# Francis-Rings/MotionEditor

Measured on AMD Instinct MI355X. Metric: denoise-steps/sec, 24f x 512^2 two-branch UNet3D+ControlNet(+adapter+K/V injection), higher is better.
Workload: dtype f16

## Files before the change

motioneditor_amd/csrc/gemm.hip:

```cpp
#include "me_common.h"
#include "../../include/motioned.h"
#include <stdio.h>
#include <stdlib.h>

namespace {

constexpr int BK = 64;
#ifndef WIDE_TERMS
#define WIDE_TERMS 0
#endif
constexpr int STAGE_REG = 0, STAGE_GLDS = 1, STAGE_BUF = 2;
constexpr int ROWEPI_FLAG = 1 << 30, TILEORDER_FLAG = 1 << 29;

template <bool NT = false>
__device__ __forceinline__ void st16(f16* p, uint4 v) {
  if constexpr (NT) {
    typedef unsigned u32x4 __attribute__((ext_vector_type(4)));
    __builtin_nontemporal_store((u32x4){v.x, v.y, v.z, v.w}, reinterpret_cast<u32x4*>(p));
  } else {
    *reinterpret_cast<uint4*>(p) = v;
  }
}
template <bool NT = false>
__device__ __forceinline__ void st8(f16* p, uint2 v) {
// ... 770 lines not shown
    const int wrows = min(a.N - n0, BN);
    const auto wsrd = __builtin_amdgcn_make_buffer_rsrc(const_cast<f16*>(W + (long)n0 * wtaps * a.K), 0, (unsigned)(((long)(wrows - 1) * wtaps + taps) * a.K * 2), 0x00020000);
    unsigned xo[XROWS], wo[WROWS];
#pragma unroll
    for (int i = 0; i < WROWS; ++i) wo[i] = (unsigned)(((long)(srow + RSTR * i) * wtaps * a.K + scol) * 2);
    auto set_tap_off = [&](int tap) {
#pragma unroll
      for (int i = 0; i < XROWS; ++i) {
        const int sr = src_row(a, rinfo[i], tap, ups3);
        xo[i] = sr < 0 ? OOB : (unsigned)(((long)(sr - brow) * a.ldx + scol) * 2);
      }
    };
    int tap_l = it0 / nkc, kc_l = it0 - (it0 / nkc) * nkc;
    set_tap_off(tap_l);
    auto gload = [&](int buf) {
      char* dx = reinterpret_cast<char*>(sX + buf * BM * LD) + wave * 1024;
      char* dw = reinterpret_cast<char*>(sW + buf * BN * LD) + wave * 1024;
      const int sx = kc_l * (BK * 2), sw = (tap_l * a.K + kc_l * BK) * 2;
#pragma unroll
      for (int i = 0; i < XROWS; ++i) __builtin_amdgcn_raw_ptr_buffer_load_lds(xsrd, (lptr_t)(dx + i * (RSTR * 128)), 16, (int)xo[i], sx, 0, 0);
#pragma unroll
      for (int i = 0; i < WROWS; ++i) __builtin_amdgcn_raw_ptr_buffer_load_lds(wsrd, (lptr_t)(dw + i * (RSTR * 128)), 16, (int)wo[i], sw, 0, 0);
      if (++kc_l == nkc) {
        kc_l = 0;
        if (++tap_l < taps) set_tap_off(tap_l);
      }
    };
    gload(0);
    __syncthreads();
    for (int it = it0; it < it1; ++it) {
      const int buf = (it - it0) & 1;
      if (it + 1 < it1) gload(buf ^ 1);
      compute(buf);
      __syncthreads();
    }
    if (S > 1) {
      float* wk = reinterpret_cast<float*>(a.work) + (long)blockIdx.y * a.M * a.N;
#pragma unroll
      for (int i = 0; i < MT; ++i) {
        const int m = m0 + wm * WM + i * 16 + (lane & 15);
        if (m >= a.M) continue;
#pragma unroll
        for (int j = 0; j < NT; ++j) {
          const int n = n0 + wn * WN + j * 16 + (lane >> 4) * 4;
          if (n < a.N) *reinterpret_cast<f32x4*>(wk + (long)m * a.N + n) = acc[j][i];
        }
      }
      return;
    }
  } else if constexpr (STAGE == STAGE_GLDS) {
    typedef const __attribute__((address_space(1))) void* gptr_t;
    typedef __attribute__((address_space(3))) void* lptr_t;
    const f16* zsrc = reinterpret_cast<const f16*>(&g_zero16);
    auto gload = [&](int it, int buf) {
      int tap = it / nkc;
      int c = (it - tap * nkc) * BK + scol;
      bool kok = c < a.K;
      long wk = (long)tap * a.K + c;
      if (packk) {
        wk = it * BK + scol;
        tap = (int)wk / a.K;
        c = (int)wk - tap * a.K;
        kok = tap < 9;
        if (!kok) tap = 8;
      }
      set_tap(tap);
      char* dx = reinterpret_cast<char*>(sX + buf * BM * LD) + wave * 1024;
      char* dw = reinterpret_cast<char*>(sW + buf * BN * LD) + wave * 1024;
#pragma unroll
      for (int i = 0; i < XROWS; ++i) {
        const f16* src = (kok && xoff[i] >= 0) ? X + xoff[i] + c : zsrc;
        __builtin_amdgcn_global_load_lds((gptr_t)src, (lptr_t)(dx + i * (RSTR * 128)), 16, 0, 0);
      }
#pragma unroll
      for (int i = 0; i < WROWS; ++i) {
        const int n = n0 + srow + RSTR * i;
        const f16* src = (kok && n < a.N) ? W + (long)n * wtaps * a.K + wk : zsrc;
        __builtin_amdgcn_global_load_lds((gptr_t)src, (lptr_t)(dw + i * (RSTR * 128)), 16, 0, 0);
      }
    };
    gload(0, 0);
    __syncthreads();
    for (int it = 0; it < nit; ++it) {
      const int buf = it & 1;
      if (it + 1 < nit) gload(it + 1, buf ^ 1);
      compute(buf);
      __syncthreads();
    }
  } else {
    uint4 rx[XROWS], rw[WROWS];
    auto gload = [&](int it) {
      const int tap = it / nkc;
      const int c = (it - tap * nkc) * BK + scol;
      set_tap(tap);
      const bool kok = c < a.K;
#pragma unroll
      for (int i = 0; i < XROWS; ++i) rx[i] = (kok && xoff[i] >= 0) ? ldg128(X + xoff[i] + c) : zero128();
#pragma unroll
      for (int i = 0; i < WROWS; ++i) {
        const int n = n0 + srow + RSTR * i;
        rw[i] = (kok && n < a.N) ? ldg128(W + ((long)n * wtaps + tap) * a.K + c) : zero128();
      }
    };
    auto sstore = [&](int buf) {
      f16* dx = sX + buf * BM * LD;
      f16* dw = sW + buf * BN * LD;
#pragma unroll
      for (int i = 0; i < XROWS; ++i) *reinterpret_cast<uint4*>(dx + (srow + RSTR * i) * LD + scol) = rx[i];
#pragma unroll
      for (int i = 0; i < WROWS; ++i) *reinterpret_cast<uint4*>(dw + (srow + RSTR * i) * LD + scol) = rw[i];
    };
    gload(0);
    sstore(0);
    __syncthreads();
    for (int it = 0; it < nit; ++it) {
      const int buf = it & 1;
      if (it + 1 < nit) gload(it + 1);
      compute(buf);
      if (it + 1 < nit) sstore(buf ^ 1);
      __syncthreads();
    }
  }

  if (a.ln_stats) ln_fold_acc<NT, MT>(a, acc, m0 + wm * WM, n0 + wn * WN, lane);
  const int ncols = a.geglu ? BN / 2 : BN;
  const int Nout = a.geglu ? a.N / 2 : a.N;
  constexpr bool CFITS = (size_t)BM * (BN + 8) <= (size_t)2 * (BM + BN) * LD;
  const bool wide_store = CFITS && (Nout % 8 == 0) && (a.ldc % 8 == 0) && ((reinterpret_cast<uintptr_t>(a.C) & 15) == 0) && !a.C2 && !ups3;
  auto rowfn = [&](int i) {
    const int m = m0 + wm * WM + i * 16 + (lane & 15);
    if (m >= a.M) return -1;
    return ups3 ? out_row(a, make_row(a, m, par, true), par) : m;
  };
  if (!wide_store) {
    epilogue<NT, MT, WN>(a, acc, rowfn, m0, n0, wn, lane, nullptr, 0);
    return;
  }
  constexpr int CLD = BN + 8;
  f16* sC = reinterpret_cast<f16*>(smem);
  epilogue<NT, MT, WN>(a, acc, rowfn, m0, n0, wn, lane, sC, CLD);
  __syncthreads();
  f16* C = reinterpret_cast<f16*>(a.C);
  const int vpr = ncols / 8;
  const int nb0 = a.geglu ? n0 / 2 : n0;
  for (int idx = tid; idx < BM * vpr; idx += NTHR) {
    const int row = idx / vpr, c8 = (idx - row * vpr) * 8;
    const int m = m0 + row, n = nb0 + c8;
    if (m < a.M && n < Nout) *reinterpret_cast<uint4*>(C + (long)m * a.ldc + n) = *reinterpret_cast<const uint4*>(sC + row * CLD + c8);
  }
}

constexpr int HALO_W = 18, HALO_ROWS = HALO_W * HALO_W, HALO_INSTR = (HALO_ROWS + 7) / 8;
constexpr int HALO_BYTES = HALO_INSTR * 1024, CONVW_BYTES = 320 * 128;

__global__ __launch_bounds__(512, 2) void conv3_halo_kernel(const me_gemm_args a) {
  constexpr int BN = 320, WN = 160, NT = 10, MT = 4;
  extern __shared__ __attribute__((aligned(16))) char smem[];
  char* sH = smem;
  char* sWt = smem + HALO_BYTES;

  const int tid = threadIdx.x;
  const int lane = tid & 63;
  const int wave = __builtin_amdgcn_readfirstlane(tid >> 6);
  const int wm = wave >> 1, wn = wave & 1;

  const int nbn = a.N / BN;
  const int tx_n = a.Win >> 4, ppi = tx_n * (a.Hin >> 4);
  const int hw = a.Hin * a.Win;
  const int w = xcd_remap(blockIdx.x, (a.M / hw) * ppi * nbn);
  const int tile_n = w % nbn, patch = w / nbn;
  const int img = patch / ppi, pr = patch - img * ppi;
  const int ty = pr / tx_n, tx = pr - ty * tx_n;
  const int y0 = ty * 16, x0 = tx * 16, n0 = tile_n * BN;

  const f16* __restrict__ X = reinterpret_cast<const f16*>(a.X);
  const f16* __restrict__ W = reinterpret_cast<const f16*>(a.W);

  const int srow = wave * 8 + (lane >> 3);
  const int scol = ((lane & 7) ^ ((4 * (wave & 1) + (lane >> 4)) & 7)) * 8;
  typedef __attribute__((address_space(3))) void* lptr_t;
  constexpr unsigned OOB = 0x80000000u;
  const auto xsrd = __builtin_amdgcn_make_buffer_rsrc(const_cast<f16*>(X + (long)img * hw * a.ldx), 0, OOB, 0x00020000);
  const auto wsrd = __builtin_amdgcn_make_buffer_rsrc(const_cast<f16*>(W + (long)n0 * 9 * a.K), 0, (unsigned)((long)BN * 9 * a.K * 2), 0x00020000);
  unsigned hoff[6];
#pragma unroll
  for (int i = 0; i < 6; ++i) {
    const int hr = srow + 64 * i;
    unsigned o = OOB;
    if (hr < HALO_ROWS) {
      const int hy = hr / HALO_W, hx = hr - hy * HALO_W;
      const int iy = y0 - 1 + hy, ix = x0 - 1 + hx;
      if (iy >= 0 && iy < a.Hin && ix >= 0 && ix < a.Win) o = (unsigned)(((long)(iy * a.Win + ix) * a.ldx + scol) * 2);
    }
    hoff[i] = o;
  }
  auto load_halo = [&](int kc) {
#pragma unroll
    for (int i = 0; i < 6; ++i) {
      if (wave + 8 * i < HALO_INSTR)
        __builtin_amdgcn_raw_ptr_buffer_load_lds(xsrd, (lptr_t)(sH + (wave + 8 * i) * 1024), 16, (int)hoff[i], kc * (BK * 2), 0, 0);
    }
  };
  unsigned woff[5];
#pragma unroll
  for (int i = 0; i < 5; ++i) woff[i] = (unsigned)(((long)(srow + 64 * i) * 9 * a.K + scol) * 2);
  auto load_w = [&](int tap, int kc, int buf) {
    char* dw = sWt + buf * CONVW_BYTES + wave * 1024;
    const int so = (tap * a.K + kc * BK) * 2;
#pragma unroll
    for (int i = 0; i < 5; ++i) __builtin_amdgcn_raw_ptr_buffer_load_lds(wsrd, (lptr_t)(dw + i * 8192), 16, (int)woff[i], so, 0, 0);
  };

  f32x4 acc[NT][MT];
  init_acc<NT, MT, WN>(a, acc, n0, wn, lane);

  const int frow = lane & 15, fg = lane >> 4;
  auto compute = [&](int tap, int buf) {
    const int ky = tap / 3, kx = tap - ky * 3;
    const char* bw = sWt + buf * CONVW_BYTES;
    const int hbase = (wm * 4 + ky) * HALO_W + kx + frow;
#pragma unroll
    for (int ks = 0; ks < BK / 32; ++ks) {
      f16x8 fx[MT], fw[NT];
#pragma unroll
      for (int i = 0; i < MT; ++i) {
        const int row = hbase + i * HALO_W;
        fx[i] = *reinterpret_cast<const f16x8*>(sH + row * 128 + (((ks * 4 + fg) ^ ((row >> 1) & 7)) << 4));
      }
#pragma unroll
      for (int j = 0; j < NT; ++j) {
        const int row = wn * WN + j * 16 + frow;
        fw[j] = *reinterpret_cast<const f16x8*>(bw + row * 128 + (((ks * 4 + fg) ^ ((row >> 1) & 7)) << 4));
      }
#pragma unroll
      for (int j = 0; j < NT; ++j)
#pragma unroll
        for (int i = 0; i < MT; ++i) acc[j][i] = mfma16(fw[j], fx[i], acc[j][i]);
    }
  };

  const int nkc = a.K / BK;
  load_halo(0);
  load_w(0, 0, 0);
  __syncthreads();
  int it = 0;
  for (int kc = 0; kc < nkc; ++kc) {
    for (int tap = 0; tap < 9; ++tap, ++it) {
      const int buf = it & 1;
      const bool last_tap = tap == 8;
      if (!last_tap) load_w(tap + 1, kc, buf ^ 1);
      else if (kc + 1 < nkc) load_w(0, kc + 1, buf ^ 1);
      compute(tap, buf);
      if (last_tap && kc + 1 < nkc) {
        __syncthreads();
        load_halo(kc + 1);
      }
      __syncthreads();
    }
  }

  auto rowfn = [&](int i) { return img * hw + (y0 + wm * 4 + i) * a.Win + x0 + (lane & 15); };
  epilogue<NT, MT, WN>(a, acc, rowfn, 0, n0, wn, lane, nullptr, 0);
}

template <int BM, int BN, bool GATHER, int EPI, bool UPS3 = false>
__global__ __launch_bounds__(512, 2) void gemm8p_kernel(const me_gemm_args a) {
  static_assert(!UPS3 || (GATHER && BN == 320 && EPI <= 0), "ups 3: gather kernels, term-free row pass or direct epilogues");
  constexpr int WN = BN / 4, NT = WN / 16, NT0 = (NT + 1) / 2, NT1 = NT / 2;
  constexpr int GR = BM / 2, HALF = GR / 2, MH = HALF / 16, MT = 2 * MH;
  constexpr int NPA = 2 * HALF / 8;
  constexpr int ABYTES = BM * 128, BUFBYTES = (BM + BN) * 128;
  static_assert(BN % 64 == 0 && NT1 >= 1 && HALF % 16 == 0 && NPA >= 8 && NPA <= 16, "wave tile");
  extern __shared__ __attribute__((aligned(16))) char smem[];

  const int tid = threadIdx.x;
  const int lane = tid & 63;
  const int wave = __builtin_amdgcn_readfirstlane(tid >> 6);
  const int wr = wave >> 2, wc = wave & 3;

  const int nbn = (a.N + BN - 1) / BN;
  const int nbm = (a.M - a.m_off + BM - 1) / BM;
  constexpr bool ups3 = UPS3;
  const int nbmp = ups3 ? 4 * nbm : nbm;
  const int w = xcd_remap(blockIdx.x, nbmp * nbn);
  int tile_n, tile_m;
  if (a.splits_ & TILEORDER_FLAG) { tile_m = w % nbmp; tile_n = w / nbmp; }
  else { tile_n = w % nbn; tile_m = w / nbn; }
  const int par = ups3 ? tile_m / nbm : 0;
  tile_m -= par * nbm;
  const int m0 = a.m_off + tile_m * BM, n0 = tile_n * BN;

  const f16* __restrict__ X = reinterpret_cast<const f16*>(a.X);
  const int taps = !GATHER ? 1 : (a.gather == ME_GATHER_CONV3 ? (ups3 ? 4 : 9) : (a.gather == ME_GATHER_TCONV ? 3 : 1));
  const int wtaps = ups3 ? 16 : taps;
  const f16* __restrict__ W = reinterpret_cast<const f16*>(a.W) + (long)(4 * par) * a.K;
  const int nkc = a.K / BK;
  const int nit = taps * nkc;

  typedef __attribute__((address_space(3))) void* lptr_t;
  constexpr unsigned OOB = 0x80000000u;
  long brow = m0;
  if (GATHER) {
    if (a.gather == ME_GATHER_CONV3) brow = (long)(m0 / (ups3 ? a.Hin * a.Win : a.Hout * a.Wout)) * a.Hin * a.Win;
    else if (a.gather == ME_GATHER_TCONV) brow = m0 > a.npix ? m0 - a.npix : 0;
  }
  const auto xsrd = __builtin_amdgcn_make_buffer_rsrc(const_cast<f16*>(X + brow * a.ldx), 0, OOB, 0x00020000);
  const int wrows = min(a.N - n0, BN);
  const auto wsrd = __builtin_amdgcn_make_buffer_rsrc(const_cast<f16*>(W + (long)n0 * wtaps * a.K), 0, (unsigned)(((long)(wrows - 1) * wtaps + taps) * a.K * 2), 0x00020000);

  const int prow = lane >> 3;
  const int scol = ((lane & 7) ^ ((4 * (wave & 1) + (lane >> 4)) & 7)) * 8;
  int rA[2][2], rB0[NT0], rB1[NT1];
#pragma unroll
  for (int i = 0; i < 2; ++i) {
    const int p = wave + 8 * i;
    rA[0][i] = __builtin_amdgcn_readfirstlane((p / (HALF / 8)) * GR + 8 * (p % (HALF / 8)));
    rA[1][i] = __builtin_amdgcn_readfirstlane((p / (HALF / 8)) * GR + HALF + 8 * (p % (HALF / 8)));
  }
  const bool two_a = __builtin_amdgcn_readfirstlane(wave + 8 < NPA ? 1 : 0) != 0;
#pragma unroll
  for (int i = 0; i < NT0; ++i) {
    const int p = wave + 8 * i;
    rB0[i] = __builtin_amdgcn_readfirstlane((p / (2 * NT0)) * WN + 8 * (p % (2 * NT0)));
  }
#pragma unroll
  for (int i = 0; i < NT1; ++i) {
    const int p = wave + 8 * i;
    rB1[i] = __builtin_amdgcn_readfirstlane((p / (2 * NT1)) * WN + 16 * NT0 + 8 * (p % (2 * NT1)));
  }

  unsigned* tab = reinterpret_cast<unsigned*>(smem + 2 * BUFBYTES);
  unsigned xo[2][2];
  if constexpr (GATHER) {
    const int r = tid & 255;
    const RowInfo ri = make_row(a, r < BM ? m0 + r : a.M, par, ups3);
    for (int tap = tid >> 8; tap < taps; tap += 2) {
      const int sr = src_row(a, ri, tap, ups3);
      tab[tap * 256 + r] = sr < 0 ? OOB : (unsigned)((long)(sr - brow) * a.ldx * 2);
    }
    if (ups3 && tid < 256) tab[4 * 256 + r] = ri.valid ? (unsigned)out_row(a, ri, par) : ~0u;
    __syncthreads();
  } else {
#pragma unroll
    for (int h = 0; h < 2; ++h)
#pragma unroll
      for (int i = 0; i < 2; ++i) {
        const int m = m0 + rA[h][i] + prow;
        xo[h][i] = (m < a.M && (i == 0 || two_a)) ? (unsigned)(((long)(m - brow) * a.ldx + scol) * 2) : OOB;
      }
  }
  unsigned wo0[NT0], wo1[NT1];
#pragma unroll
  for (int i = 0; i < NT0; ++i) wo0[i] = (unsigned)(((long)(rB0[i] + prow) * wtaps * a.K + scol) * 2);
#pragma unroll
  for (int i = 0; i < NT1; ++i) wo1[i] = (unsigned)(((long)(rB1[i] + prow) * wtaps * a.K + scol) * 2);

  struct Cur { int tap, kc, tl; };
  Cur cA0 = {0, 0, 0}, cA1 = {0, 0, 0};
  int tB0 = 0, tB1 = 0;
  auto issueA = [&](Cur& c, int half) {
    char* base = smem + (c.tl & 1) * BUFBYTES;
    const int sx = __builtin_amdgcn_readfirstlane((GATHER ? c.kc : c.tl) * (BK * 2));
    const bool live = c.tl < nit;
    unsigned v[2];
#pragma unroll
    for (int i = 0; i < 2; ++i) {
      if constexpr (GATHER) v[i] = tab[__builtin_amdgcn_readfirstlane(min(c.tap, taps - 1)) * 256 + min(rA[half][i] + prow, 255)] + (unsigned)(scol * 2);
      else v[i] = xo[half][i];
    }
    __builtin_amdgcn_raw_ptr_buffer_load_lds(xsrd, (lptr_t)(base + rA[half][0] * 128), 16, (int)(live ? v[0] : OOB), sx, 0, 0);
    if (BM == 256 || two_a) __builtin_amdgcn_raw_ptr_buffer_load_lds(xsrd, (lptr_t)(base + rA[half][1] * 128), 16, (int)(live ? v[1] : OOB), sx, 0, 0);
    ++c.tl;
    if constexpr (GATHER) {
      if (++c.kc == nkc) { c.kc = 0; ++c.tap; }
    }
  };
  auto issueB0 = [&]() {
    char* base = smem + (tB0 & 1) * BUFBYTES + ABYTES;
    const int sw = __builtin_amdgcn_readfirstlane(tB0 * (BK * 2));
    const bool live = tB0 < nit;
#pragma unroll
    for (int i = 0; i < NT0; ++i)
      __builtin_amdgcn_raw_ptr_buffer_load_lds(wsrd, (lptr_t)(base + rB0[i] * 128), 16, (int)(live ? wo0[i] : OOB), sw, 0, 0);
    ++tB0;
  };
  auto issueB1 = [&]() {
    char* base = smem + (tB1 & 1) * BUFBYTES + ABYTES;
    const int sw = __builtin_amdgcn_readfirstlane(tB1 * (BK * 2));
    const bool live = tB1 < nit;
#pragma unroll
    for (int i = 0; i < NT1; ++i)
      __builtin_amdgcn_raw_ptr_buffer_load_lds(wsrd, (lptr_t)(base + rB1[i] * 128), 16, (int)(live ? wo1[i] : OOB), sw, 0, 0);
    ++tB1;
  };

  f32x4 acc[NT][MT];
  init_acc<NT, MT, WN>(a, acc, n0, wc, lane);

  const int frow = lane & 15, fg = lane >> 4;
  const int c0 = (fg ^ ((frow >> 1) & 7)) << 4;
  const int la0 = (wr * GR + frow) * 128 + c0, la1 = la0 ^ 64;
  const int lb0 = ABYTES + (wc * WN + frow) * 128 + c0, lb1 = lb0 ^ 64;
  f16x8 fa[2][MH], fb[2][NT0];
  auto readA = [&](int buf, int half) {
#pragma unroll
    for (int i = 0; i < MH; ++i) {
      fa[0][i] = *reinterpret_cast<const f16x8*>(smem + buf * BUFBYTES + la0 + (half * MH + i) * 2048);
      fa[1][i] = *reinterpret_cast<const f16x8*>(smem + buf * BUFBYTES + la1 + (half * MH + i) * 2048);
    }
  };
  auto readB = [&](int buf, int j0, int nj) {
#pragma unroll
    for (int j = 0; j < NT0; ++j) {
      if (j < nj) {
        fb[0][j] = *reinterpret_cast<const f16x8*>(smem + buf * BUFBYTES + lb0 + (j0 + j) * 2048);
// ... 258 lines not shown
  const char* e = getenv("ME_GEMM_8P_128");
  const long v = e ? atol(e) : 192;
  return v > 0 ? v : (1L << 60);
}

long geglu_min_tiles() {
  const char* e = getenv("ME_GEMM_GEGLU_MIN");
  return e ? atol(e) : 240;
}

int min_ktiles_192() {
  const char* e = getenv("ME_GEMM_192_MINK");
  return e ? atoi(e) : 4;
}

long n64_below() {
  const char* e = getenv("ME_GEMM_N64_BELOW");
  return e ? atol(e) : 200;
}

bool tile160() {
  static int on = -1;
  if (on < 0) {
    const char* e = getenv("ME_GEMM_TILE160");
    on = (e && e[0] == '0') ? 0 : 1;
  }
  return on == 1;
}

}

extern "C" void me_set_error(const char* msg);
extern "C" void me_set_kernel(const char* name);
extern "C" const char* me_last_kernel(void);

static thread_local bool g_ln_fused = false;

template <int BM, int BN, int STAGE, int WM = 64, bool UPS3 = false>
static int launch_gemm(const me_gemm_args* a, hipStream_t st) {
  const size_t lds = (size_t)2 * (BM + BN) * (STAGE != STAGE_REG ? BK : BK + 8) * sizeof(f16);
  static bool attr_set_dev[64] = {};
  int dev_id = 0;
  (void)hipGetDevice(&dev_id);
  bool& attr_set = attr_set_dev[dev_id & 63];
  if (!attr_set) {
    if (hipFuncSetAttribute(reinterpret_cast<const void*>(&gemm_kernel<BM, BN, STAGE, WM, UPS3>), hipFuncAttributeMaxDynamicSharedMemorySize, (int)lds) != hipSuccess) {
      me_set_error("me_gemm: hipFuncSetAttribute(MaxDynamicSharedMemorySize) failed");
      return ME_EHIP;
    }
    attr_set = true;
  }
  constexpr int pm = UPS3 ? 4 : 1;
  if (UPS3 != (a->gather == ME_GATHER_CONV3 && a->ups == 3)) { me_set_error("me_gemm: internal: ups = 3 launch on the wrong instantiation"); return ME_EINVAL; }
  const int nbm = (a->M - a->m_off + BM - 1) / BM * pm, nbn = (a->N + BN - 1) / BN;
  (void)hipGetLastError();
  me_gemm_args b = *a;
  b.splits_ = 0;
  int S = 1;
  if (STAGE == STAGE_BUF && a->work) {
    const int nit = (a->K / 64) * (a->gather == ME_GATHER_CONV3 ? 9 : (a->gather == ME_GATHER_TCONV ? 3 : 1));
    const int Msel = a->sel_rows > a->M ? a->sel_rows : a->M;
    S = choose_split(a, (long)((Msel + BM - 1) / BM) * nbn, nit);
    if ((int64_t)S * a->M * a->N * 4 > a->work_bytes || a->N % 4 || ((uintptr_t)a->work & 15)) S = 1;
  }
  if (S > 1) {
    b.splits_ = S;
    hipLaunchKernelGGL((gemm_kernel<BM, BN, STAGE, WM, UPS3>), dim3(nbm * nbn, S), dim3(BM / WM * 128), lds, st, b);
    const long vec = (long)a->M * (a->N / 4);
    hipLaunchKernelGGL(gemm_splitk_reduce_kernel, dim3((unsigned)((vec + 255) / 256 < 4096 ? (vec + 255) / 256 : 4096)), dim3(256), 0, st, b);
  } else {
    hipLaunchKernelGGL((gemm_kernel<BM, BN, STAGE, WM, UPS3>), dim3(nbm * nbn), dim3(BM / WM * 128), lds, st, b);
  }
  {
    char nm[64];
    snprintf(nm, sizeof(nm), "gemm_kernel<%d,%d%s>%s", BM, BN, STAGE == STAGE_REG ? ",reg" : "", S > 1 ? "+splitk" : "");
    me_set_kernel(nm);
  }
  if (hipGetLastError() != hipSuccess) {
    me_set_error("me_gemm: kernel launch failed");
    return ME_EHIP;
  }
  return ME_OK;
}

template <int BM, int BN, bool GATHER, int EPI, bool UPS3 = false>
static int launch_gemm8p_epi(const me_gemm_args& b, hipStream_t st) {
  const int lds = 2 * (BM + BN) * 128 + (GATHER ? 9 * 256 * 4 : (EPI == 0 ? LN_LDS_BYTES : 0));
  static bool attr_set_dev[64] = {};
  int dev_id = 0;
  (void)hipGetDevice(&dev_id);
  bool& attr_set = attr_set_dev[dev_id & 63];
  if (!attr_set) {
    if (hipFuncSetAttribute(reinterpret_cast<const void*>(&gemm8p_kernel<BM, BN, GATHER, EPI, UPS3>), hipFuncAttributeMaxDynamicSharedMemorySize, lds) != hipSuccess) {
      me_set_error("me_gemm: hipFuncSetAttribute(MaxDynamicSharedMemorySize) failed");
      return ME_EHIP;
    }
    attr_set = true;
  }
  constexpr int pm = UPS3 ? 4 : 1;
  const int nbm = (b.M - b.m_off + BM - 1) / BM * pm, nbn = (b.N + BN - 1) / BN;
  hipLaunchKernelGGL((gemm8p_kernel<BM, BN, GATHER, EPI, UPS3>), dim3(nbm * nbn), dim3(512), lds, st, b);
  return ME_OK;
}

template <int BM, int BN, bool GATHER>
static int launch_gemm8p(const me_gemm_args* a, hipStream_t st) {
  (void)hipGetLastError();
  me_gemm_args b = *a;
  b.splits_ = 0;
  int epi = -1;
  {
    auto al = [](const void* p, int ld) { return p == nullptr || (ld % 8 == 0 && (reinterpret_cast<uintptr_t>(p) & 15) == 0); };
    const int f = (a->rowvec ? 2 : 0) | (a->res ? 4 : 0) | (a->res2 ? 8 : 0);
    const bool ups3 = a->gather == ME_GATHER_CONV3 && a->ups == 3;
    if (BN == 320 && !(ups3 && f != 0) && row_epilogue() && !a->geglu && a->act == 0 && a->N % 320 == 0 && (f == 0 || f == 2 || f == 4 || f == 6 || f == 12) && al(a->C, a->ldc) &&
        al(a->rowvec, a->ldrv) && al(a->res, a->ldr) && al(a->res2, a->ldr2) && (!a->C2 || f == 0))
      epi = f;
    if (tile_order_exp()) b.splits_ |= TILEORDER_FLAG;
    if (BN == 256 && BM == 256 && row_epilogue() && a->geglu && a->N % 256 == 0 && al(a->C, a->ldc) && !a->C2) epi = 0;
    if (epi >= 0) b.splits_ |= ROWEPI_FLAG;
    g_ln_fused = BN == 320 && epi >= 0 && a->ln_out != nullptr;
    if (!g_ln_fused) b.ln_out = nullptr;
  }
  int rc;
  const bool ups3_launch = a->gather == ME_GATHER_CONV3 && a->ups == 3;
  if (ups3_launch) {
    if constexpr (GATHER && BN == 320) rc = epi == 0 ? launch_gemm8p_epi<BM, BN, true, 0, true>(b, st) : launch_gemm8p_epi<BM, BN, true, -1, true>(b, st);
    else { me_set_error("me_gemm: internal: ups = 3 launch on a kernel without the mode"); return ME_EINVAL; }
  } else if constexpr (BN == 256) {
    rc = epi == 0 ? launch_gemm8p_epi<BM, BN, GATHER, 0>(b, st) : launch_gemm8p_epi<BM, BN, GATHER, -1>(b, st);
  } else {
    switch (epi) {
      case 0: rc = launch_gemm8p_epi<BM, BN, GATHER, 0>(b, st); break;
      case 2: rc = launch_gemm8p_epi<BM, BN, GATHER, 2>(b, st); break;
      case 4: rc = launch_gemm8p_epi<BM, BN, GATHER, 4>(b, st); break;
      case 6: rc = launch_gemm8p_epi<BM, BN, GATHER, 6>(b, st); break;
      case 12: rc = launch_gemm8p_epi<BM, BN, GATHER, 12>(b, st); break;
      default: rc = launch_gemm8p_epi<BM, BN, GATHER, -1>(b, st); break;
    }
  }
  if (rc != ME_OK) return rc;
  {
    char nm[64];
    snprintf(nm, sizeof(nm), "gemm8p_kernel<%d,%d,%s>", BM, BN, GATHER ? "true" : "false");
    me_set_kernel(nm);
  }
  if (hipGetLastError() != hipSuccess) {
    me_set_error("me_gemm: kernel launch failed");
    return ME_EHIP;
  }
  return ME_OK;
}

static int launch_conv_halo(const me_gemm_args* a, hipStream_t st) {
  const int lds = HALO_BYTES + 2 * CONVW_BYTES;
  static bool attr_set_dev[64] = {};
  int dev_id = 0;
  (void)hipGetDevice(&dev_id);
  bool& attr_set = attr_set_dev[dev_id & 63];
  if (!attr_set) {
    if (hipFuncSetAttribute(reinterpret_cast<const void*>(&conv3_halo_kernel), hipFuncAttributeMaxDynamicSharedMemorySize, lds) != hipSuccess) {
      me_set_error("me_gemm: hipFuncSetAttribute(MaxDynamicSharedMemorySize) failed");
      return ME_EHIP;
    }
    attr_set = true;
  }
  const long blocks = (long)(a->M / 256) * (a->N / 320);
  (void)hipGetLastError();
  hipLaunchKernelGGL(conv3_halo_kernel, dim3((unsigned)blocks), dim3(512), lds, st, *a);
  me_set_kernel("conv3_halo_kernel");
  if (hipGetLastError() != hipSuccess) {
    me_set_error("me_gemm: kernel launch failed");
    return ME_EHIP;
  }
  return ME_OK;
}

extern "C" int64_t me_gemm_work_bytes(const me_gemm_args* a) {
  if (!a || a->M <= 0 || a->N <= 0 || a->K <= 0 || a->geglu || a->K % 64 || a->N % 4) return 0;
  const int nit = (a->K / 64) * (a->gather == ME_GATHER_CONV3 ? 9 : (a->gather == ME_GATHER_TCONV ? 3 : 1));
  const long blocks = (long)((a->M + 127) / 128) * ((a->N + 159) / 160);
  const int S = choose_split(a, blocks, nit);
  return S > 1 ? (int64_t)4 * a->M * a->N * 4 : 0;
}

static int gemm_dispatch(const me_gemm_args* a, void* stream);

extern "C" int me_gemm(const me_gemm_args* a, void* stream) {
  if (!a || !a->X || !a->W || !a->C) { me_set_error("me_gemm: null pointer"); return ME_EINVAL; }
  if (a->ln_stats) {
    if (a->gather != ME_GATHER_DENSE || a->bias || a->alpha != 1.0f || a->rowvec || a->res || a->res2 || a->act || !a->ln_colsum || !a->ln_cvec || a->ln_parts < 1 || a->ln_parts > 4 || a->ln_stride < 2 * (int64_t)a->M ||
        (a->ln_stride & 1) || ((uintptr_t)a->ln_stats & 7) || (((uintptr_t)a->ln_colsum | (uintptr_t)a->ln_cvec) & 15) || !(a->ln_eps > 0.f)) {
      me_set_error("me_gemm: a LayerNorm-folded launch is dense, has no bias (it is inside ln_cvec), no rowvec / residual / activation and alpha == 1; ln_colsum / ln_cvec fp32 [N] 16-byte aligned, "
                   "ln_stats 8-byte aligned with 1 <= ln_parts <= 4 parts ln_stride >= 2 M floats apart, ln_eps > 0");
      return ME_EINVAL;
    }
  }
  if (a->ln_out && (a->geglu || a->C2 || a->N % 8 || a->N > 1536 || a->ldc % 8 || ((uintptr_t)a->C & 15) || ((uintptr_t)a->ln_out & 7) || a->ln_out_stride < 2 * (int64_t)a->M || (a->ln_out_stride & 1))) {
    me_set_error("me_gemm: ln_out needs a plain fp16 output of N % 8 == 0, N <= 1536 columns (no GEGLU, no head-major panels), ldc % 8 == 0, and parts >= 2 M floats apart");
    return ME_EINVAL;
  }
  g_ln_fused = false;
  const int rc = gemm_dispatch(a, stream);
  if (rc != ME_OK || !a->ln_out || g_ln_fused) return rc;
  char nm[96];
  snprintf(nm, sizeof(nm), "%s", me_last_kernel());
  const int rc2 = me_ln_stats(reinterpret_cast<const f16*>(a->C) + (long)a->m_off * a->ldc, a->ldc, (int64_t)a->M - a->m_off, a->N,
                              reinterpret_cast<float*>(a->ln_out) + 2 * (long)a->m_off, a->ln_out_stride, stream);
  me_set_kernel(nm);
  return rc2;
}

static int gemm_dispatch(const me_gemm_args* a, void* stream) {
  if (a->M <= 0 || a->N <= 0 || a->K <= 0) { me_set_error("me_gemm: non-positive dimension"); return ME_EINVAL; }
  if (a->K % 8 || a->ldx % 8 || a->ldc % 4 || a->N % 4) { me_set_error("me_gemm: K, ldx must be multiples of 8 and N, ldc of 4"); return ME_EINVAL; }
  if (((uintptr_t)a->X | (uintptr_t)a->W) & 15 || ((uintptr_t)a->C & 7)) { me_set_error("me_gemm: misaligned pointer"); return ME_EINVAL; }
  if (a->gather < 0 || a->gather > 2) { me_set_error("me_gemm: bad gather mode"); return ME_EINVAL; }
  if (a->gather == ME_GATHER_CONV3) {
    if (a->Hin <= 0 || a->Win <= 0 || a->Hout <= 0 || a->Wout <= 0 || (a->stride != 1 && a->stride != 2) || a->ups < 0 || a->ups > 3 ||
        (a->pad0 != 0 && a->pad0 != 1) || a->M % (a->Hout * a->Wout)) { me_set_error("me_gemm: bad conv geometry"); return ME_EINVAL; }
    if (a->ups == 3 && (a->stride != 1 || a->pad0 || a->Hout != 2 * a->Hin || a->Wout != 2 * a->Win || a->geglu)) {
      me_set_error("me_gemm: ups = 3 (folded nearest 2x) needs stride 1, pad0 = 0, Hout = 2 Hin, Wout = 2 Win and weights [N, 16, K]");
      return ME_EINVAL;
    }
  }
  if (a->gather == ME_GATHER_TCONV) {
    const int ftot = a->frames_total > 0 ? a->frames_total : a->frames;
    if (a->frames <= 0 || a->npix <= 0 || a->chunk <= 0 || ftot % a->chunk || (a->m_off == 0 && a->sel_rows <= a->M && a->M % (a->frames * a->npix)) || a->frame0 < 0 ||
        a->frame0 + a->frames > ftot) { me_set_error("me_gemm: bad tconv geometry"); return ME_EINVAL; }
  }
  if (a->rowvec && (a->rows_per_vec <= 0 || a->ldrv % 4 || ((uintptr_t)a->rowvec & 7))) { me_set_error("me_gemm: bad rowvec"); return ME_EINVAL; }
  if (a->res && (a->ldr % 4 || ((uintptr_t)a->res & 7))) { me_set_error("me_gemm: bad residual"); return ME_EINVAL; }
  if (a->res2 && (a->ldr2 % 4 || ((uintptr_t)a->res2 & 7))) { me_set_error("me_gemm: bad second residual"); return ME_EINVAL; }
  if (a->res_rows < 0 || a->res2_rows < 0) { me_set_error("me_gemm: negative res_rows"); return ME_EINVAL; }
  if (a->act < 0 || a->act > 2) { me_set_error("me_gemm: bad activation"); return ME_EINVAL; }
  if (a->bias && ((uintptr_t)a->bias & 7)) { me_set_error("me_gemm: misaligned bias"); return ME_EINVAL; }
  if (a->geglu && (a->N % 32 || a->rowvec || a->res || a->res2 || a->act || a->alpha != 1.0f)) { me_set_error("me_gemm: geglu needs N % 32 == 0, alpha == 1 and no rowvec/res/act"); return ME_EINVAL; }
  if (a->m_off < 0 || a->m_off >= a->M || (a->m_off > 0 && a->gather == ME_GATHER_CONV3)) { me_set_error("me_gemm: m_off must lie in [0, M) and is for dense / TemporalConv launches"); return ME_EINVAL; }
  if (a->C2 && (a->geglu || a->act || a->rowvec || a->res || a->res2 || a->c2_dh <= 0 || a->c2_dh % 8 || a->c2_col0 < 0 || a->c2_col0 % 16 || a->c2_col0 >= a->N ||
                (a->N - a->c2_col0) % a->c2_dh || a->c2_hs % 8 || a->c2_hs < (int64_t)a->M * a->c2_dh || ((uintptr_t)a->C2 & 15) || a->gather == ME_GATHER_CONV3)) {
    me_set_error("me_gemm: head-major output (C2) needs a term-free epilogue, c2_dh % 8 == 0, c2_col0 % 16 == 0, whole heads, c2_hs % 8 == 0 and >= M * c2_dh, 16-byte alignment");
    return ME_EINVAL;
  }
  hipStream_t st = reinterpret_cast<hipStream_t>(stream);
  me_gemm_args par_args;
  const int pm = a->gather == ME_GATHER_CONV3 && a->ups == 3 ? 4 : 1;
  if (pm == 4) {
    par_args = *a;
    par_args.M = a->M / 4;
    par_args.sel_rows = a->sel_rows / 4;
    par_args.ln_out = nullptr;
    a = &par_args;
  }
#define ME_LAUNCH_GEMM(BM_, BN_, STAGE_) (pm == 4 ? launch_gemm<BM_, BN_, STAGE_, 64, true>(a, st) : launch_gemm<BM_, BN_, STAGE_>(a, st))
  const bool wide = a->N % 128 == 0 || a->N % 64 != 0;
  if (stage_impl() == STAGE_GLDS || pm == 4) {
    const int Msel = a->sel_rows > a->M ? a->sel_rows : a->M;
    const long big_blocks = (long)((Msel + 255) / 256) * pm * (a->N / 320);
    if (a->gather == ME_GATHER_CONV3 && a->stride == 1 && a->ups == 0 && !a->pad0 && a->N % 320 == 0 && a->K % 64 == 0 && a->Hin % 16 == 0 &&
        a->Win % 16 == 0 && !a->geglu && big_blocks >= halo_min_blocks() && conv_halo())
      return launch_conv_halo(a, st);
    const bool buf = a->K % 64 == 0 && buf_stage();
    const int nit8 = (a->K / 64) * (a->gather == ME_GATHER_CONV3 ? (pm == 4 ? 4 : 9) : (a->gather == ME_GATHER_TCONV ? 3 : 1));
    const bool dense = a->gather == ME_GATHER_DENSE;
    if (a->geglu && dense && buf && use_8p() > 0 && nit8 >= use_8p() && a->N % 256 == 0 && (long)((Msel + 255) / 256) * (a->N / 256) >= geglu_min_tiles())
      return launch_gemm8p<256, 256, false>(a, st);
    if (a->N % 320 == 0 && big_blocks >= big_min_blocks()) {
      if (buf && use_8p() > 0 && nit8 >= use_8p()) {
        if (!a->geglu) return dense ? launch_gemm8p<256, 320, false>(a, st) : launch_gemm8p<256, 320, true>(a, st);
        if (dense && a->N % 256 == 0 && (long)((Msel + 255) / 256) * (a->N / 256) >= big_min_blocks()) return launch_gemm8p<256, 256, false>(a, st);
      }
      return buf ? ME_LAUNCH_GEMM(256, 320, STAGE_BUF) : ME_LAUNCH_GEMM(256, 320, STAGE_GLDS);
    }
    if (a->N % 320 == 0 && !a->geglu && buf && use_8p() > 0 && nit8 >= min_ktiles_192() && nit8 >= use_8p() && (long)((Msel + 191) / 192) * pm * (a->N / 320) >= min_tiles_192())
      return dense ? launch_gemm8p<192, 320, false>(a, st) : launch_gemm8p<192, 320, true>(a, st);
    if (dense && a->N % 320 == 0 && !a->geglu && buf && use_8p() > 0 && nit8 >= min_ktiles_192() && nit8 >= use_8p() && (long)((Msel + 127) / 128) * (a->N / 320) >= min_tiles_128())
      return launch_gemm8p<128, 320, false>(a, st);
    const long blocks160 = (long)((Msel + 127) / 128) * pm * ((a->N + 159) / 160);
    {
      const long blocks128 = (long)((Msel + 127) / 128) * pm * ((a->N + 127) / 128);
      if (a->N % 64 == 0 && blocks128 < n64_below()) return buf ? ME_LAUNCH_GEMM(128, 64, STAGE_BUF) : ME_LAUNCH_GEMM(128, 64, STAGE_GLDS);
    }
    if (a->N % 128 == 0 && blocks160 < 512) return buf ? ME_LAUNCH_GEMM(128, 128, STAGE_BUF) : ME_LAUNCH_GEMM(128, 128, STAGE_GLDS);
    if (!a->geglu && a->N % 160 == 0 && tile160()) return buf ? ME_LAUNCH_GEMM(128, 160, STAGE_BUF) : ME_LAUNCH_GEMM(128, 160, STAGE_GLDS);
    if (wide) return buf ? ME_LAUNCH_GEMM(128, 128, STAGE_BUF) : ME_LAUNCH_GEMM(128, 128, STAGE_GLDS);
    return ME_LAUNCH_GEMM(128, 64, STAGE_GLDS);
  }
#undef ME_LAUNCH_GEMM
  return wide ? launch_gemm<128, 128, STAGE_REG>(a, st) : launch_gemm<128, 64, STAGE_REG>(a, st);
}
```

Measured before the change: 6.822.

## Add pipelined halo prefetch and specialized row epilogues to the conv3 halo kernel

After: 6.835 (median of 6 runs). No clear change (+0.2%).

```diff
diff --git a/motioneditor_amd/csrc/gemm.hip b/motioneditor_amd/csrc/gemm.hip
--- a/motioneditor_amd/csrc/gemm.hip
+++ b/motioneditor_amd/csrc/gemm.hip
@@ -946,12 +946,16 @@
 
 constexpr int HALO_W = 18, HALO_ROWS = HALO_W * HALO_W, HALO_INSTR = (HALO_ROWS + 7) / 8;
 constexpr int HALO_BYTES = HALO_INSTR * 1024, CONVW_BYTES = 320 * 128;
-
+constexpr int HALO_LATE = 4, HALO_EARLY = HALO_INSTR - HALO_LATE;
+constexpr int HALO_PIPE_BYTES = (HALO_LATE + 2 * HALO_EARLY) * 1024;
+static_assert(HALO_LATE * 8 <= 2 * HALO_W && HALO_EARLY <= 5 * 8 && HALO_PIPE_BYTES + 2 * CONVW_BYTES <= 160 * 1024, "halo pipeline: late pieces below halo row 36, five taps of early pieces, LDS of a CU");
+
+template <bool PIPE, int EPI>
 __global__ __launch_bounds__(512, 2) void conv3_halo_kernel(const me_gemm_args a) {
   constexpr int BN = 320, WN = 160, NT = 10, MT = 4;
   extern __shared__ __attribute__((aligned(16))) char smem[];
   char* sH = smem;
-  char* sWt = smem + HALO_BYTES;
+  char* sWt = smem + (PIPE ? HALO_PIPE_BYTES : HALO_BYTES);
 
   const int tid = threadIdx.x;
   const int lane = tid & 63;
@@ -971,29 +975,39 @@
   const f16* __restrict__ W = reinterpret_cast<const f16*>(a.W);
 
   const int srow = wave * 8 + (lane >> 3);
+  auto hpiece = [&](int i) { return PIPE ? (i == 0 ? wave : HALO_LATE + wave + 8 * (i - 1)) : wave + 8 * i; };
+  auto hvalid = [&](int i) { return PIPE && i == 0 ? wave < HALO_LATE : hpiece(i) < HALO_INSTR; };
   const int scol = ((lane & 7) ^ ((4 * (wave & 1) + (lane >> 4)) & 7)) * 8;
   typedef __attribute__((address_space(3))) void* lptr_t;
   constexpr unsigned OOB = 0x80000000u;
   const auto xsrd = __builtin_amdgcn_make_buffer_rsrc(const_cast<f16*>(X + (long)img * hw * a.ldx), 0, OOB, 0x00020000);
   const auto wsrd = __builtin_amdgcn_make_buffer_rsrc(const_cast<f16*>(W + (long)n0 * 9 * a.K), 0, (unsigned)((long)BN * 9 * a.K * 2), 0x00020000);
-  unsigned hoff[6];
-#pragma unroll
-  for (int i = 0; i < 6; ++i) {
-    const int hr = srow + 64 * i;
+  auto halo_off = [&](int hr) {
     unsigned o = OOB;
     if (hr < HALO_ROWS) {
       const int hy = hr / HALO_W, hx = hr - hy * HALO_W;
       const int iy = y0 - 1 + hy, ix = x0 - 1 + hx;
       if (iy >= 0 && iy < a.Hin && ix >= 0 && ix < a.Win) o = (unsigned)(((long)(iy * a.Win + ix) * a.ldx + scol) * 2);
     }
-    hoff[i] = o;
-  }
+    return o;
+  };
+  unsigned hoff[PIPE ? 1 : 6];
+  if constexpr (!PIPE) {
+#pragma unroll
+    for (int i = 0; i < 6; ++i) hoff[i] = halo_off(srow + 64 * i);
+  }
+  auto hplace = [&](int i, int par) { return sH + (i == 0 ? wave : hpiece(i) + par * HALO_EARLY) * 1024; };
   auto load_halo = [&](int kc) {
 #pragma unroll
     for (int i = 0; i < 6; ++i) {
-      if (wave + 8 * i < HALO_INSTR)
-        __builtin_amdgcn_raw_ptr_buffer_load_lds(xsrd, (lptr_t)(sH + (wave + 8 * i) * 1024), 16, (int)hoff[i], kc * (BK * 2), 0, 0);
-    }
+      if (hvalid(i))
+        __builtin_amdgcn_raw_ptr_buffer_load_lds(xsrd, (lptr_t)(PIPE ? hplace(i, kc & 1) : sH + (wave + 8 * i) * 1024), 16, (int)(PIPE ? halo_off(hpiece(i) * 8 + (lane >> 3)) : hoff[PIPE ? 0 : i]), kc * (BK * 2), 0, 0);
+    }
+  };
+  auto load_halo_part = [&](int tap, int kc) {
+    const int i = tap < 5 ? tap + 1 : 0;
+    if ((tap < 5 || tap == 6) && hvalid(i))
+      __builtin_amdgcn_raw_ptr_buffer_load_lds(xsrd, (lptr_t)hplace(i, kc & 1), 16, (int)halo_off(hpiece(i) * 8 + (lane >> 3)), kc * (BK * 2), 0, 0);
   };
   unsigned woff[5];
 #pragma unroll
@@ -1009,7 +1023,7 @@
   init_acc<NT, MT, WN>(a, acc, n0, wn, lane);
 
   const int frow = lane & 15, fg = lane >> 4;
-  auto compute = [&](int tap, int buf) {
+  auto compute = [&](int tap, int buf, int hpar) {
     const int ky = tap / 3, kx = tap - ky * 3;
     const char* bw = sWt + buf * CONVW_BYTES;
     const int hbase = (wm * 4 + ky) * HALO_W + kx + frow;
@@ -1019,7 +1033,8 @@
 #pragma unroll
       for (int i = 0; i < MT; ++i) {
         const int row = hbase + i * HALO_W;
-        fx[i] = *reinterpret_cast<const f16x8*>(sH + row * 128 + (((ks * 4 + fg) ^ ((row >> 1) & 7)) << 4));
+        const int hp = PIPE && row >= HALO_LATE * 8 ? hpar : 0;
+        fx[i] = *reinterpret_cast<const f16x8*>(sH + hp + row * 128 + (((ks * 4 + fg) ^ ((row >> 1) & 7)) << 4));
       }
 #pragma unroll
       for (int j = 0; j < NT; ++j) {
@@ -1038,23 +1053,39 @@
   load_w(0, 0, 0);
   __syncthreads();
   int it = 0;
-  for (int kc = 0; kc < nkc; ++kc) {
-    for (int tap = 0; tap < 9; ++tap, ++it) {
-      const int buf = it & 1;
-      const bool last_tap = tap == 8;
-      if (!last_tap) load_w(tap + 1, kc, buf ^ 1);
-      else if (kc + 1 < nkc) load_w(0, kc + 1, buf ^ 1);
-      compute(tap, buf);
-      if (last_tap && kc + 1 < nkc) {
+  if constexpr (PIPE) {
+#pragma unroll 1
+    for (int kc = 0; kc < nkc; ++kc) {
+#pragma unroll 1
+      for (int tap = 0; tap < 9; ++tap, ++it) {
+        const int buf = it & 1;
+        if (tap != 8) load_w(tap + 1, kc, buf ^ 1);
+        else if (kc + 1 < nkc) load_w(0, kc + 1, buf ^ 1);
+        if (kc + 1 < nkc) load_halo_part(tap, kc + 1);
+        compute(tap, buf, (kc & 1) * (HALO_EARLY * 1024));
         __syncthreads();
-        load_halo(kc + 1);
-      }
-      __syncthreads();
+      }
+    }
+  } else {
+    for (int kc = 0; kc < nkc; ++kc) {
+      for (int tap = 0; tap < 9; ++tap, ++it) {
+        const int buf = it & 1;
+        const bool last_tap = tap == 8;
+        if (!last_tap) load_w(tap + 1, kc, buf ^ 1);
+        else if (kc + 1 < nkc) load_w(0, kc + 1, buf ^ 1);
+        compute(tap, buf, 0);
+        if (last_tap && kc + 1 < nkc) {
+          __syncthreads();
+          load_halo(kc + 1);
+        }
+        __syncthreads();
+      }
     }
   }
 
   auto rowfn = [&](int i) { return img * hw + (y0 + wm * 4 + i) * a.Win + x0 + (lane & 15); };
-  epilogue<NT, MT, WN>(a, acc, rowfn, 0, n0, wn, lane, nullptr, 0);
+  if constexpr (EPI >= 0) epilogue_rows<EPI, NT, MT, WN>(a, acc, rowfn, 0, n0, wn, lane, nullptr, 0);
+  else epilogue<NT, MT, WN>(a, acc, rowfn, 0, n0, wn, lane, nullptr, 0);
 }
 
 template <int BM, int BN, bool GATHER, int EPI, bool UPS3 = false>
@@ -1619,14 +1650,15 @@
   return ME_OK;
 }
 
-static int launch_conv_halo(const me_gemm_args* a, hipStream_t st) {
-  const int lds = HALO_BYTES + 2 * CONVW_BYTES;
+template <bool PIPE, int EPI>
+static int launch_conv_halo_pipe(const me_gemm_args* a, hipStream_t st) {
+  const int lds = (PIPE ? HALO_PIPE_BYTES : HALO_BYTES) + 2 * CONVW_BYTES;
   static bool attr_set_dev[64] = {};
   int dev_id = 0;
   (void)hipGetDevice(&dev_id);
   bool& attr_set = attr_set_dev[dev_id & 63];
   if (!attr_set) {
-    if (hipFuncSetAttribute(reinterpret_cast<const void*>(&conv3_halo_kernel), hipFuncAttributeMaxDynamicSharedMemorySize, lds) != hipSuccess) {
+    if (hipFuncSetAttribute(reinterpret_cast<const void*>(&conv3_halo_kernel<PIPE, EPI>), hipFuncAttributeMaxDynamicSharedMemorySize, lds) != hipSuccess) {
       me_set_error("me_gemm: hipFuncSetAttribute(MaxDynamicSharedMemorySize) failed");
       return ME_EHIP;
     }
@@ -1634,13 +1666,27 @@
   }
   const long blocks = (long)(a->M / 256) * (a->N / 320);
   (void)hipGetLastError();
-  hipLaunchKernelGGL(conv3_halo_kernel, dim3((unsigned)blocks), dim3(512), lds, st, *a);
+  hipLaunchKernelGGL(conv3_halo_kernel<PIPE, EPI>, dim3((unsigned)blocks), dim3(512), lds, st, *a);
   me_set_kernel("conv3_halo_kernel");
   if (hipGetLastError() != hipSuccess) {
     me_set_error("me_gemm: kernel launch failed");
     return ME_EHIP;
   }
   return ME_OK;
+}
+
+static int launch_conv_halo(const me_gemm_args* a, hipStream_t st) {
+  const char* e = getenv("ME_CONV_HALO_PIPE");
+  if (e && e[0] == '1') return launch_conv_halo_pipe<true, -1>(a, st);
+  const int f = (a->geglu || a->act != 0) ? -1 : ((a->rowvec ? 2 : 0) | (a->res ? 4 : 0) | (a->res2 ? 8 : 0));
+  const char* g = getenv("ME_CONV_HALO_EPI");
+  if (g && g[0] == '0') return launch_conv_halo_pipe<false, -1>(a, st);
+  switch (f) {
+    case 0: return launch_conv_halo_pipe<false, 0>(a, st);
+    case 2: return launch_conv_halo_pipe<false, 2>(a, st);
+    case 4: return launch_conv_halo_pipe<false, 4>(a, st);
+    default: return launch_conv_halo_pipe<false, -1>(a, st);
+  }
 }
 
 extern "C" int64_t me_gemm_work_bytes(const me_gemm_args* a) {
```
